# jthorborg/signalizer

Hardware: AMD Instinct MI355X
Metric: 32768-pt stereo STFT frames/sec (75% overlap); achieved HBM GB/s vs peak (higher is better)
Workload: dtype f32

## Files before the change

signalizer_amd/csrc/fft_scalar.hpp:

```cpp
#pragma once
#include "fft_common.hpp"

namespace sgz {

__device__ __forceinline__ v2 cmulScalar(v2 c, float2 w)
{
    const float t0 = c.x * w.x, t1 = c.x * w.y;
    return v2{__builtin_fmaf(-c.y, w.y, t0), __builtin_fmaf(c.y, w.x, t1)};
}
__device__ __forceinline__ float2 cmulScalar(float2 c, float2 w)
{
    const float t0 = c.x * w.x, t1 = c.x * w.y;
    return float2{__builtin_fmaf(-c.y, w.y, t0), __builtin_fmaf(c.y, w.x, t1)};
}
__device__ __forceinline__ float2 csqScalar(float2 w)
{
    const float d = w.x * w.x;
    return float2{__builtin_fmaf(-w.y, w.y, d), (w.x + w.x) * w.y};
}

template <int LR, int S, int BASE, int NREG>
__device__ __forceinline__ void ditStage(v2 (&c)[NREG])
{
    constexpr int n = 1 << LR, m = 1 << S, h = m / 2;
#pragma unroll
    for (int k0 = 0; k0 < n; k0 += m) {
#pragma unroll
        for (int j = 0; j < h; ++j) {
            const int ia = BASE + brev(k0 + j, LR), ib = BASE + brev(k0 + j + h, LR);
            const v2 a = c[ia], b = c[ib];
            const int tw = j * (32 / m);
            if (tw == 0) { c[ia] = a + b; c[ib] = a - b; }
            else if (tw == 8) { c[ia] = v2{a.x + b.y, a.y - b.x}; c[ib] = v2{a.x - b.y, a.y + b.x}; }
            else if (tw < 8) {
                const float cs = cos32(tw), sn = sin32(tw);
                const float pr = __builtin_fmaf(b.y, sn, __builtin_fmaf(b.x, cs, a.x));
                const float pi = __builtin_fmaf(b.x, -sn, __builtin_fmaf(b.y, cs, a.y));
                c[ia] = v2{pr, pi};
                c[ib] = v2{__builtin_fmaf(2.f, a.x, -pr), __builtin_fmaf(2.f, a.y, -pi)};
            } else {
                const float cs = cos32(tw - 8), sn = sin32(tw - 8);
                const float pr = __builtin_fmaf(b.x, -sn, __builtin_fmaf(b.y, cs, a.x));
                const float pi = __builtin_fmaf(b.y, -sn, __builtin_fmaf(b.x, -cs, a.y));
                c[ia] = v2{pr, pi};
                c[ib] = v2{__builtin_fmaf(2.f, a.x, -pr), __builtin_fmaf(2.f, a.y, -pi)};
            }
        }
    }
}

template <int LR, int BASE, int NREG, int FIRST = 1>
__device__ __forceinline__ void ditScalar(v2 (&c)[NREG])
{
    if constexpr (FIRST <= 1) ditStage<LR, 1, BASE>(c);
    if constexpr (FIRST <= 2 && LR >= 2) ditStage<LR, 2, BASE>(c);
    if constexpr (LR >= 3) ditStage<LR, 3, BASE>(c);
    if constexpr (LR >= 4) ditStage<LR, 4, BASE>(c);
    if constexpr (LR >= 5) ditStage<LR, 5, BASE>(c);
}

__device__ __forceinline__ void bflyPackedLow(v2 &a, v2 &b, v2 k)
{
    v2 t, p, q;
    asm("v_pk_fma_f32 %0, %1, %2, %3 op_sel_hi:[1,0,1]" : "=v"(t) : "v"(b), "s"(k), "v"(a));
    asm("v_pk_fma_f32 %0, %1, %2, %3 op_sel:[1,1,0] op_sel_hi:[0,1,1] neg_hi:[1,0,0]" : "=v"(p) : "v"(b), "s"(k), "v"(t));
    asm("v_pk_fma_f32 %0, %1, 2.0, %2 op_sel_hi:[1,0,1] neg_lo:[0,0,1] neg_hi:[0,0,1]" : "=v"(q) : "v"(a), "v"(p));
    a = p; b = q;
}
__device__ __forceinline__ void bflyPackedHigh(v2 &a, v2 &b, v2 k)
{
    v2 t, p, q;
    asm("v_pk_fma_f32 %0, %1, %2, %3 op_sel:[1,0,0] op_sel_hi:[0,0,1] neg_hi:[1,0,0]" : "=v"(t) : "v"(b), "s"(k), "v"(a));
    asm("v_pk_fma_f32 %0, %1, %2, %3 op_sel:[0,1,0] op_sel_hi:[1,1,1] neg_lo:[1,0,0] neg_hi:[1,0,0]" : "=v"(p) : "v"(b), "s"(k), "v"(t));
    asm("v_pk_fma_f32 %0, %1, 2.0, %2 op_sel_hi:[1,0,1] neg_lo:[0,0,1] neg_hi:[0,0,1]" : "=v"(q) : "v"(a), "v"(p));
    a = p; b = q;
}
__device__ __forceinline__ void bflyPackedRot(v2 &a, v2 &b)
{
    v2 p, q;
    asm("v_pk_add_f32 %0, %1, %2 op_sel:[0,1] op_sel_hi:[1,0] neg_hi:[0,1]" : "=v"(p) : "v"(a), "v"(b));
    asm("v_pk_add_f32 %0, %1, %2 op_sel:[0,1] op_sel_hi:[1,0] neg_lo:[0,1]" : "=v"(q) : "v"(a), "v"(b));
    a = p; b = q;
}

template <bool UNIT_A>
__device__ __forceinline__ void bflyPackedFusedTw(v2 &a, v2 &b, v2 ta, v2 tb)
{
    v2 u = a, t, p, q;
    if constexpr (!UNIT_A) {
        v2 m;
        asm("v_pk_mul_f32 %0, %1, %2 op_sel:[0,0] op_sel_hi:[1,0]" : "=v"(m) : "v"(a), "v"(ta));
        asm("v_pk_fma_f32 %0, %1, %2, %3 op_sel:[1,1,0] op_sel_hi:[0,1,1] neg_lo:[1,0,0]" : "=v"(u) : "v"(a), "v"(ta), "v"(m));
    }
    asm("v_pk_fma_f32 %0, %1, %2, %3 op_sel:[0,0,0] op_sel_hi:[1,0,1]" : "=v"(t) : "v"(b), "v"(tb), "v"(u));
    asm("v_pk_fma_f32 %0, %1, %2, %3 op_sel:[1,1,0] op_sel_hi:[0,1,1] neg_lo:[1,0,0]" : "=v"(p) : "v"(b), "v"(tb), "v"(t));
    asm("v_pk_fma_f32 %0, %1, 2.0, %2 op_sel_hi:[1,0,1] neg_lo:[0,0,1] neg_hi:[0,0,1]" : "=v"(q) : "v"(u), "v"(p));
    a = p; b = q;
}

template <int LR, int S, int BASE, int NREG>
__device__ __forceinline__ void ditStagePacked(v2 (&c)[NREG])
{
    constexpr int n = 1 << LR, m = 1 << S, h = m / 2;
#pragma unroll
    for (int k0 = 0; k0 < n; k0 += m) {
#pragma unroll
        for (int j = 0; j < h; ++j) {
            const int ia = BASE + brev(k0 + j, LR), ib = BASE + brev(k0 + j + h, LR);
            const int tw = j * (32 / m);
            if (tw == 0) { const v2 a = c[ia], b = c[ib]; c[ia] = a + b; c[ib] = a - b; }
            else if (tw == 8) bflyPackedRot(c[ia], c[ib]);
            else if (tw < 8) bflyPackedLow(c[ia], c[ib], v2{cos32(tw), sin32(tw)});
            else bflyPackedHigh(c[ia], c[ib], v2{cos32(tw - 8), sin32(tw - 8)});
        }
    }
}
template <int LR, int BASE, int NREG, int FIRST = 1>
__device__ __forceinline__ void ditPacked(v2 (&c)[NREG])
{
    if constexpr (FIRST <= 1) ditStagePacked<LR, 1, BASE>(c);
    if constexpr (FIRST <= 2 && LR >= 2) ditStagePacked<LR, 2, BASE>(c);
    if constexpr (LR >= 3) ditStagePacked<LR, 3, BASE>(c);
    if constexpr (LR >= 4) ditStagePacked<LR, 4, BASE>(c);
    if constexpr (LR >= 5) ditStagePacked<LR, 5, BASE>(c);
}

}
```

signalizer_amd/csrc/spectrum_real.hip:

```cpp
#include <algorithm>

#include "real_common.hpp"

#ifdef SGZ_DEBUG
#define RCLK(slot)                                                                                                     \
    do {                                                                                                               \
        if (prm.phaseClock && (tid & 63) == 0 && unit == long(prm.clkUnit)) prm.phaseClock[16 * (tid >> 6) + (slot)] = __builtin_readcyclecounter(); \
    } while (0)
#define RTRACE(which)                                                                                                  \
    do {                                                                                                               \
        if (prm.phaseClock && prm.clkUnit == 0xffffu && tid == 0) {                                                    \
            unsigned long long *t = prm.phaseClock + 256 + 4 * unit;                                                   \
            t[which] = __builtin_amdgcn_s_memrealtime();                                                               \
            if (which == 0) { t[2] = __builtin_amdgcn_s_getreg(4 | (31 << 11)); t[3] = __builtin_amdgcn_s_getreg(20 | (31 << 11)) | (static_cast<unsigned long long>(blockIdx.x) << 32); } \
        }                                                                                                              \
    } while (0)
#else
#define RCLK(slot) do { } while (0)
#define RTRACE(which) do { } while (0)
#endif

namespace sgz {

template <int R1, int LR1, int BASE, int Q = 0>
__device__ __forceinline__ void e1WriteRun(uint32_t wa, const v2 (&c)[32])
{
    if constexpr (Q < R1) { ldsWrite64<(Q & 15) * 512 * 8>(wa + uint32_t(Q >> 4) * 65536u, c[BASE + brev(Q, LR1)]); e1WriteRun<R1, LR1, BASE, Q + 1>(wa, c); }
}

template <int R1, int LR1, int Q = 0>
__device__ __forceinline__ void e1WritePairRun(uint32_t wa, const v2 (&c)[32])
{
    if constexpr (Q < R1) { ldsWrite128<(Q & 15) * 512 * 8>(wa + uint32_t(Q >> 4) * 65536u, c[brev(Q, LR1)], c[R1 + brev(Q, LR1)]); e1WritePairRun<R1, LR1, Q + 1>(wa, c); }
}

template <int R, int R1, int U, int LR1, int u = 0>
__device__ __forceinline__ void pass1Columns(v2 (&c)[R])
{
    if constexpr (u < U) {
        ditPacked<LR1, u * R1>(c);
        pass1Columns<R, R1, U, LR1, u + 1>(c);
    }
}

constexpr float kRotA1Cm1 = -0x1.3bd3ccp-24f, kRotA1Sin = 0x1.921fb4p-12f;
constexpr float kRotA4Cm1 = -0x1.3bd3c8p-20f, kRotA4Sin = 0x1.921faap-10f;
__device__ __forceinline__ float4 rotatePhaseForward(const float4 ph, const float cm1, const float sn)
{
    const v2 pc = v2{ph.x, ph.y}, ps = v2{ph.z, ph.w};
    const v2 kc = v2{cm1, cm1}, ks = v2{sn, sn};
    const v2 c2 = __builtin_elementwise_fma(pc, kc, __builtin_elementwise_fma(ps, -ks, pc));
    const v2 s2 = __builtin_elementwise_fma(ps, kc, __builtin_elementwise_fma(pc, ks, ps));
    return float4{c2.x, c2.y, s2.x, s2.y};
}
__device__ __forceinline__ float2 rotateTwiddle(const float2 w, const float cm1, const float sn)
{
    const v2 v = v2{w.x, w.y}, sw = v2{w.y, w.x};
    const v2 r = __builtin_elementwise_fma(v, v2{cm1, cm1}, __builtin_elementwise_fma(sw, v2{sn, -sn}, v));
    return float2{r.x, r.y};
}

__device__ __forceinline__ void windowPairCos(v2 &lo, v2 &hi, const int a32, const v2 pc, const v2 ps, const v2 p0)
{
    v2 t = pc;
    if (a32 != 0) {
        const v2 k = v2{cos32(a32), sin32(a32)};
        v2 m;
        asm("v_pk_mul_f32 %0, %1, %2 op_sel:[0,1] op_sel_hi:[1,1]" : "=v"(m) : "v"(ps), "s"(k));
        asm("v_pk_fma_f32 %0, %1, %2, %3 op_sel:[0,0,0] op_sel_hi:[1,0,1] neg_lo:[0,0,1] neg_hi:[0,0,1]" : "=v"(t) : "v"(pc), "s"(k), "v"(m));
    }
    v2 wa, wb;
    asm("v_pk_add_f32 %0, %1, %2" : "=v"(wa) : "v"(t), "s"(p0));
    asm("v_pk_add_f32 %0, %1, %2 neg_lo:[1,0] neg_hi:[1,0]" : "=v"(wb) : "v"(t), "s"(p0));
    lo = lo * wa;
    hi = hi * wb;
}

template <int LR1, int MIX, typename P>
__device__ __forceinline__ void realMapSettle(const P &prm, float *lds, const int tid, const int side, const long task, const long self,
                                              const ChunkTables &tb, ChunkMap<(1 << (LR1 + 5))> &mapper, float *re, float *ce, float *spec)
{
    constexpr int R = 32, R1 = 1 << LR1, T = R1 * R, M = R1 * R * R, N = 2 * M;
    constexpr bool MONO = MIX == 1 || MIX == 3;
    const ChannelIndex at{N, side ? M : 0};
    [[maybe_unused]] const long unit = MONO ? task : self;
    if (prm.binsOut) {
        float *dst = prm.binsOut + size_t(task) * (N + 1) + (side ? M : 0);
        for (int i = tid; i <= M; i += T)
            if (MONO || i != (side ? 0 : M)) dst[i] = lds[chunkPos(i)];
    }
    if (!MONO && (prm.lowCount[0] + prm.lowCount[1]) && tid < kLowBins) prm.low[size_t(self) * kLowBins + tid] = lds[at(side ? N - tid : tid)];
    RCLK(8);
    mapper.run(tb, at, lds, re, ce, prm.invSize, tid);
    RCLK(9);
    RTRACE(1);
    if (MONO) {
        if (prm.mapped && prm.lowCount[0]) {
            float *out = prm.mapped + size_t(task) * prm.P;
            for (uint32_t i = tid; i < prm.lowCount[0]; i += T) {
                const uint32_t x = prm.lowPixels[i];
                out[x] = complexDcPixel(prm.recsFull[x], prm.weights, prm.invSize, N, prm.mode,
                                        [&](int k) { return k >= N ? 0.f : lds[chunkPos(k)]; },
                                        [&](int sl) { return make_float2(spec[2 * sl], spec[2 * sl + 1]); });
            }
        }
        return;
    }
}

[[maybe_unused]] __device__ __forceinline__ void setWavePriority(const uint32_t p)
{
    if (p != 0u) { if (p == 1u) __builtin_amdgcn_s_setprio(1); else if (p == 2u) __builtin_amdgcn_s_setprio(2); else __builtin_amdgcn_s_setprio(3); }
}

constexpr uint32_t kNyHopRows = 4;
template <int LR1, bool PRIO, bool SHARE>
__device__ __forceinline__ void nyquistUnit(const RealParams &prm, float *lds, const uint32_t light, const int tid)
{
    constexpr int LR = 5, R = 32, R1 = 1 << LR1, RR = R * R;
    static_assert(LR1 == 4, "the Nyquist workgroups mirror the two-columns-per-thread form (N = 32768)");
    [[maybe_unused]] const long unit = 2 * long(light) + 1;
    RTRACE(0);
#ifdef SGZ_IMAGE_PRIO
    if constexpr (PRIO) setWavePriority(prm.prioNy);
#endif
#ifdef SGZ_SCHED_SWEEP
    for (uint32_t k = 0; k < prm.nyDelay; ++k) __builtin_amdgcn_s_sleep(16);
#endif
    const uint32_t F = prm.nyFrames, perPair = uint32_t(prm.frames) / F + (uint32_t(prm.frames) % F != 0u);
    const uint32_t pair = light / perPair, f0 = (light - pair * perPair) * F;
    const uint32_t f1 = f0 + F < uint32_t(prm.frames) ? f0 + F : uint32_t(prm.frames);
    const float *X0 = prm.planar + size_t(2 * pair + 1) * prm.chStride;
    const uint32_t lane16 = uint32_t(tid) * 16u;
    const float4 ph[2] = {ldg(prm.winPhase, lane16 * 2u), ldg(prm.winPhase + 1, lane16 * 2u)};
    const v2 p0 = v2{prm.winP0, prm.winP0};
    v2 *lds2 = reinterpret_cast<v2 *>(lds);
    auto columnSum = [&](v2 (&c)[R1], const int u) {
        const v2 pc = v2{ph[u].x, ph[u].y}, ps = v2{ph[u].z, ph[u].w};
#pragma unroll
        for (int j = 0; j < R1 / 2; ++j) windowPairCos(c[j], c[j + R1 / 2], j * (32 / R1), pc, ps, p0);
        ditPacked<LR1, 0>(c);
        lds2[2 * tid + u] = c[0];
    };
    auto tree2 = [&]() {
        if (tid < R) {
            v2 s[R];
#pragma unroll
            for (int h = 0; h < R; ++h) s[h] = lds2[tid + R * h];
            ditPacked<LR, 0>(s);
            lds2[RR + tid] = s[0];
        }
    };
    auto tree3 = [&](const uint32_t f) {
        if (tid == 0) {
            v2 s[R];
#pragma unroll
            for (int r = 0; r < R; ++r) s[r] = lds2[RR + r];
            const float4 *tab = prm.tw2Full;
#pragma unroll
            for (int i = 0; i < R / 4; ++i) {
                const float4 wa = tab[i], wb = tab[i + R / 4];
                if (i == 0) bflyPackedFusedTw<true>(s[0], s[R / 2], v2{1.f, 0.f}, v2{wb.x, wb.y});
                else bflyPackedFusedTw<false>(s[2 * i], s[2 * i + R / 2], v2{wa.x, wa.y}, v2{wb.x, wb.y});
                bflyPackedFusedTw<false>(s[2 * i + 1], s[2 * i + 1 + R / 2], v2{wa.z, wa.w}, v2{wb.z, wb.w});
            }
            ditPacked<LR, 0, R, 2>(s);
            prm.ny[((size_t(f) * prm.C + pair) << 1) | 1u] = 2.f * (s[0].x - s[0].y);
        }
    };
    constexpr uint32_t HOPROWS = kNyHopRows;
    if (SHARE && f1 - f0 > 1u && prm.hop == HOPROWS * 2u * uint32_t(RR)) {
        typedef float v4 __attribute__((ext_vector_type(4)));
        v4 raw[R1];
        {
            const float *X = X0 + size_t(f0) * prm.hop;
#pragma unroll
            for (int j = 0; j < R1; ++j) raw[j] = ldgPinned<v4>(X, uint32_t(RR * j) * 8u, lane16);
        }
        for (uint32_t f = f0; f < f1; ++f) {
#pragma unroll
            for (int u = 0; u < 2; ++u) {
                v2 c[R1];
#pragma unroll
                for (int j = 0; j < R1; ++j) c[j] = u ? v2{raw[j].z, raw[j].w} : v2{raw[j].x, raw[j].y};
                columnSum(c, u);
            }
            if (f + 1u < f1) {
                const float *X = X0 + size_t(f + 1u) * prm.hop;
#pragma unroll
                for (int j = 0; j < R1 - int(HOPROWS); ++j) raw[j] = raw[j + int(HOPROWS)];
#pragma unroll
                for (int j = R1 - int(HOPROWS); j < R1; ++j) raw[j] = ldgPinned<v4>(X, uint32_t(RR * j) * 8u, lane16);
            }
            constexpr int PARK = R1 - int(HOPROWS);
            v4 *park = reinterpret_cast<v4 *>(lds + 4 * RR) + (tid & 63);
            if (__builtin_amdgcn_readfirstlane(tid) < 64) {
                __syncthreads();
#pragma unroll
                for (int j = 0; j < PARK; ++j) park[64 * j] = raw[j];
                tree2();
                __syncthreads();
                tree3(f);
#pragma unroll
                for (int j = 0; j < PARK; ++j) raw[j] = park[64 * j];
            } else {
                __syncthreads();
                __syncthreads();
            }
        }
        RTRACE(1);
        return;
    }
    for (uint32_t f = f0; f < f1; ++f) {
        const float *X = X0 + size_t(f) * prm.hop;
#pragma unroll
        for (int u = 0; u < 2; ++u) {
            v2 c[R1];
#pragma unroll
            for (int j = 0; j < R1; ++j) c[j] = ldgPinned<v2>(X, uint32_t(RR * j) * 8u + 8u * u, lane16);
            columnSum(c, u);
        }
        __syncthreads();
        tree2();
        __syncthreads();
        tree3(f);
    }
    RTRACE(1);
}

template <int LR1, bool WCOS, int MIX = 0, bool PRIO = false>
__global__ void __launch_bounds__(1 << (LR1 + 5), 4) stftRealKernel(const RealParams launchPrm)
{
    constexpr int LR = 5, R = 32, R1 = 1 << LR1, T = R1 * R, RR = R * R, M = R1 * RR, N = 2 * M, U = R / R1;
    constexpr bool MONO = MIX == 1 || MIX == 3;
    constexpr bool SIDE0 = MIX == 4;
    constexpr bool mixed = MIX == 2 || MIX == 3;
    constexpr int PADSTRIDE = chunkPos(T);
    constexpr int ROW = R + 2, TILE = R * ROW;
    constexpr int XFLOATS = realXFloats(M);
    static_assert((T / R) * TILE <= XFLOATS, "the exchange-2 tiles end below the twiddle table");
    constexpr int TAB = (XFLOATS + 3) & ~3;
    extern __shared__ __attribute__((aligned(16))) float lds[];
    const int tid0 = threadIdx.x;

    constexpr bool WALK = LR1 == 5 && MIX == 0 && WCOS;
    const uint32_t heavyUnits = SIDE0 ? uint32_t(launchPrm.frames) * launchPrm.C : gridDim.x;
    if constexpr (SIDE0) {
        if (blockIdx.x >= heavyUnits) { nyquistUnit<LR1, PRIO, PRIO>(launchPrm, lds, blockIdx.x - heavyUnits, opaque(tid0)); return; }
    }
    const uint32_t totalUnits = WALK ? uint32_t(launchPrm.frames) * launchPrm.C * 2u : heavyUnits;
    uint32_t walkIndex = blockIdx.x;
    UnitId uid = unitOfIndex<MONO || SIDE0>(launchPrm, walkIndex, totalUnits, SIDE0 && launchPrm.mateAdjacent != 0u);
    [[maybe_unused]] bool firstUnit = true;
    [[maybe_unused]] uint32_t prioEarly = 0u, prioLate = 0u, prioEnds = 0u;
    if constexpr (LR1 == 4) {
        const uint32_t cus = launchPrm.roundSize >> 1;
#ifndef SGZ_STAGGER
#define SGZ_STAGGER 5
#endif
        if (cus && !launchPrm.pipelined && gridDim.x >= 2u * cus && blockIdx.x >= cus && blockIdx.x < 2u * cus) {
#pragma unroll
            for (int k = 0; k < SGZ_STAGGER; ++k) __builtin_amdgcn_s_sleep(32);
        }
#ifdef SGZ_SCHED_SWEEP
        else if (SIDE0 && blockIdx.x >= cus) {
            for (uint32_t k = 0; k < launchPrm.mateDelay; ++k) __builtin_amdgcn_s_sleep(16);
        }
#endif
#ifndef SGZ_NO_PRIO
        if (cus && !launchPrm.pipelined && gridDim.x > 2u * cus && gridDim.x <= 3u * cus) {
#else
        if (false) {
#endif
            const uint32_t generation = blockIdx.x / cus;
            if (generation == 0u) __builtin_amdgcn_s_setprio(2); else if (generation == 1u) __builtin_amdgcn_s_setprio(1); else __builtin_amdgcn_s_setprio(3);
        }
#ifdef SGZ_IMAGE_PRIO
        if constexpr (PRIO) {
#ifdef SGZ_SCHED_SWEEP
            const uint32_t rolePrio = blockIdx.x >= cus ? launchPrm.prioMate : blockIdx.x + cus < heavyUnits ? launchPrm.prioFirst : 0u;
            const uint32_t scope = launchPrm.prioScope;
#else
            const uint32_t rolePrio = blockIdx.x >= cus ? (launchPrm.prioMate ? uint32_t(SGZ_PRIO_MATE) : 0u)
                                                        : blockIdx.x + cus < heavyUnits ? (launchPrm.prioFirst ? uint32_t(SGZ_PRIO_FIRST) : 0u) : 0u;
            constexpr uint32_t scope = SGZ_PRIO_SCOPE;
#endif
            prioEarly = (scope == 0u || scope == 3u) ? rolePrio : 0u;
            prioLate = (scope == 1u || scope == 2u) ? rolePrio : 0u;
            prioEnds = (scope & 1u) ? rolePrio : 0u;
            prioEarly = __builtin_amdgcn_readfirstlane(prioEarly); prioLate = __builtin_amdgcn_readfirstlane(prioLate); prioEnds = __builtin_amdgcn_readfirstlane(prioEnds);
        }
#endif
    }
    constexpr bool PAIRED = U == 2;
    constexpr int COLSTEP = PAIRED ? 1 : T, COLLANE = PAIRED ? 2 : 1;
    constexpr bool FRONT = LR1 >= 4 && !mixed && WCOS;
#ifdef SGZ_DIET
    constexpr bool DIET = PAIRED && FRONT && LR1 == 4;
#else
    constexpr bool DIET = false;
#endif
    [[maybe_unused]] float4 phase[U];
    [[maybe_unused]] float2 twA[U], twB[U];
    [[maybe_unused]] float4 tw2piece, tw2tail;
    v2 c[R];
    for (;;) {
    typename ParamsOf<WALK>::T &prm = *ParamsOf<WALK>::get(launchPrm);
    auto samplesOf = [&](const UnitId &u) {
        const int firstCh = MONO ? (prm.mode == SGZ_CH_RIGHT ? 1 : 0) : (mixed ? 0 : u.side);
        return prm.planar + size_t(2 * u.pair + firstCh) * prm.chStride + size_t(u.frame) * prm.hop;
    };
    auto elemOf = [&](int e) { const int u = e / R1, j = e % R1; return (PAIRED ? u : T * u) + RR * j; };
    auto requestSamples = [&](const float *X, const int tid, auto partTag) {
        constexpr int part = decltype(partTag)::value;
        const uint32_t lane8 = uint32_t(tid) * (PAIRED ? 16u : 8u);
        if constexpr (PAIRED) {
            typedef float v4 __attribute__((ext_vector_type(4)));
#pragma unroll
            for (int j = 0; j < R1; ++j) { const v4 xv = ldgPinned<v4>(X, uint32_t(RR * j) * 8u, lane8); c[j] = v2{xv.x, xv.y}; c[R1 + j] = v2{xv.z, xv.w}; }
        } else {
#pragma unroll
            for (int i = 0; i < R; ++i)
                if (part == 0 || ((i >> 3) & 1) == part - 1) c[i] = ldgPinned<v2>(X, uint32_t(elemOf(i)) * 8u, lane8);
        }
    };
    auto requestTables = [&](const int tid) {
        if constexpr (FRONT) {
            if constexpr (WALK) tw2piece = prm.tw2Full[tid < kTw2Floats / 4 ? tid : 0];
#pragma unroll
            for (int u = 0; u < (DIET ? 1 : U); ++u) {
                if (WCOS) phase[u] = ldg(prm.winPhase + COLSTEP * u, uint32_t(tid) * 16u * COLLANE);
                twA[u] = ldg(prm.tw1 + (COLSTEP * u), uint32_t(tid) * 8u * COLLANE);
                twB[u] = ldg(prm.tw1 + (COLSTEP * u + 3 * RR), uint32_t(tid) * 8u * COLLANE);
            }
            if constexpr (!WALK) { if (tid < kTw2Floats / 4) tw2piece = prm.tw2Full[tid]; }
            if (T < kTw2Floats / 4 && tid < kTw2Floats / 4 - T) tw2tail = prm.tw2Full[T + tid];
        }
    };
    if constexpr (WALK) {
        if (firstUnit) requestSamples(samplesOf(uid), tid0, std::integral_constant<int, 1>{});
        firstUnit = false;
    }
    const int tid = WALK ? opaque(tid0) : tid0;
    const int slot = tid >> 6, half = (tid >> 5) & 1, l = tid & 31, group = tid >> 5;
    const int q1 = half ? (slot == 0 ? R1 / 2 : R1 - slot) : slot;
    const int ix = half ? R - 1 - l : l;
    const uint32_t lane8 = uint32_t(tid) * (PAIRED ? 16u : 8u);
    [[maybe_unused]] const long unit = MONO ? long(uid.task) : long(uid.self);
    const int side = SIDE0 ? 0 : uid.side, pair = uid.pair;
    const long task = uid.task, frame = uid.frame, self = uid.self;

    const uint32_t maxSlots = prm.chunkSlots[0] > prm.chunkSlots[1] ? prm.chunkSlots[0] : prm.chunkSlots[1];
    const ChunkTables tb{prm.chunkEnds + side * T, prm.chunkReBase + side * T,
                         reinterpret_cast<const uint2 *>(prm.chunkRec) + size_t(side) * prm.P, prm.recs + size_t(side) * prm.P, prm.weights12,
                         prm.mapped ? prm.mapped + (size_t(task) * (MONO ? 1 : 2) + side) * prm.P : nullptr,
                         MONO ? nullptr : prm.nyBest + size_t(self) * 64, int(prm.fixFrom[side]), int(prm.P), side != 0,
#ifdef SGZ_DEBUG
                         (prm.phaseClock && unit == long(prm.clkUnit)) ? prm.phaseClock : nullptr};
#else
                         nullptr};
#endif
    const ChannelIndex at{N, side ? M : 0};
    float *re = lds + XFLOATS, *ce = re + maxSlots + 1;
    const int SCRATCH = XFLOATS + int(realExtraFloats(maxSlots, T, LR1 >= 4));
    float *spec = lds + SCRATCH + 2 * R;
    ChunkMap<T> mapper;

    RCLK(0);
    RTRACE(0);
    if constexpr (LR1 >= 4 && !FRONT) {
        for (int i = tid; i < kTw2Floats / 4; i += T) reinterpret_cast<float4 *>(lds + TAB)[i] = prm.tw2Full[i];
    }
    {
        const float *X = samplesOf(uid);
        if constexpr (WALK) {
            requestTables(tid);
            __builtin_amdgcn_sched_barrier(0);
            requestSamples(X, tid, std::integral_constant<int, 2>{});
            __builtin_amdgcn_sched_barrier(0);
            if (tid < kTw2Floats / 4) reinterpret_cast<float4 *>(lds + TAB)[tid] = tw2piece;
        } else {
            requestSamples(X, tid, std::integral_constant<int, 0>{});
            requestTables(tid);
        }
        if constexpr (FRONT) __builtin_amdgcn_sched_barrier(0);
#ifdef SGZ_IMAGE_PRIO
        if constexpr (PRIO) setWavePriority(prioEarly);
#endif
        if (mixed) {
            const float *Y = X + prm.chStride;
            const float sgn = (MONO ? prm.mode == SGZ_CH_SIDE : side == 1) ? -1.f : 1.f;
            constexpr int YB = (LR1 == 5 || (PAIRED && !WCOS)) ? 4 : 8;
#pragma unroll
            for (int b0 = 0; b0 < R; b0 += YB) {
                float2 y[YB];
#pragma unroll
                for (int i = 0; i < YB; ++i) y[i] = ldg(reinterpret_cast<const float2 *>(Y) + elemOf(b0 + i), lane8);
#pragma unroll
                for (int i = 0; i < YB; ++i) c[b0 + i] = v2{c[b0 + i].x + sgn * y[i].x, c[b0 + i].y + sgn * y[i].y};
                __builtin_amdgcn_sched_barrier(0);
            }
        }
        if (WCOS) {
            const v2 p0 = v2{prm.winP0, prm.winP0};
#pragma unroll
            for (int u = 0; u < U; ++u) {
                const float4 ph = (DIET && u == 1) ? rotatePhaseForward(phase[0], kRotA1Cm1, kRotA1Sin)
                                  : FRONT ? phase[u] : ldg(prm.winPhase + COLSTEP * u, uint32_t(tid) * 16u * COLLANE);
                const v2 pc = v2{ph.x, ph.y}, ps = v2{ph.z, ph.w};
#pragma unroll
                for (int j = 0; j < R1 / 2; ++j) {
                    constexpr int S32 = 32 / R1;
                    const int a32 = j * S32;
                    const int i = u * R1 + j, i2 = i + R1 / 2;
                    if constexpr (LR1 == 3) {
                        const float cj = cos32(a32), sj = sin32(a32);
                        const float te = a32 == 0 ? ph.x : ph.x * cj - ph.z * sj, to = a32 == 0 ? ph.y : ph.y * cj - ph.w * sj;
                        c[i] = v2{c[i].x * (prm.winP0 + te), c[i].y * (prm.winP0 + to)};
                        c[i2] = v2{c[i2].x * (prm.winP0 - te), c[i2].y * (prm.winP0 - to)};
                        continue;
                    }
                    windowPairCos(c[i], c[i2], a32, pc, ps, p0);
                }
            }
        } else {
            constexpr int B = LR1 >= 4 ? 4 : 8;
            float2 wa[B], wb[B];
#pragma unroll
            for (int i = 0; i < B; ++i) wa[i] = ldg(reinterpret_cast<const float2 *>(prm.window) + elemOf(i), lane8);
#pragma unroll
            for (int b0 = 0; b0 < R; b0 += 2 * B) {
#pragma unroll
                for (int i = 0; i < B; ++i) wb[i] = ldg(reinterpret_cast<const float2 *>(prm.window) + elemOf(b0 + B + i), lane8);
                __builtin_amdgcn_sched_barrier(0);
#pragma unroll
                for (int i = 0; i < B; ++i) { c[b0 + i] = v2{c[b0 + i].x * wa[i].x, c[b0 + i].y * wa[i].y}; asm volatile("" : "+v"(c[b0 + i])); }
                if (b0 + 2 * B < R) {
#pragma unroll
                    for (int i = 0; i < B; ++i) wa[i] = ldg(reinterpret_cast<const float2 *>(prm.window) + elemOf(b0 + 2 * B + i), lane8);
                }
                __builtin_amdgcn_sched_barrier(0);
#pragma unroll
                for (int i = 0; i < B; ++i) { c[b0 + B + i] = v2{c[b0 + B + i].x * wb[i].x, c[b0 + B + i].y * wb[i].y}; asm volatile("" : "+v"(c[b0 + B + i])); }
            }
        }
    }
    if (mixed) {
#pragma unroll
        for (int i = 0; i < R; ++i) c[i] = v2{c[i].x * 0.5f, c[i].y * 0.5f};
    }
    __builtin_amdgcn_sched_barrier(0);
    RCLK(13);
    pass1Columns<R, R1, U, LR1>(c);
#ifdef SGZ_IMAGE_PRIO
    if constexpr (PRIO) setWavePriority(prioLate);
#endif
#pragma unroll
    for (int u = 0; u < U; ++u) {
        constexpr int NB = R1 / 4 - 1;
        float2 a[3], b[NB];
        auto sq = [](float2 w) { return float2{w.x * w.x - w.y * w.y, 2.f * w.x * w.y}; };
        auto mul = [](float2 p, float2 q) { return float2{p.x * q.x - p.y * q.y, p.x * q.y + p.y * q.x}; };
        if (DIET && u == 1) {
            a[0] = rotateTwiddle(twA[0], kRotA1Cm1, kRotA1Sin);
            if (NB > 0) b[0] = rotateTwiddle(twB[0], kRotA4Cm1, kRotA4Sin);
        } else {
            a[0] = FRONT ? twA[u] : ldg(prm.tw1 + (COLSTEP * u), uint32_t(tid) * 8u * COLLANE);
            if (NB > 0) b[0] = FRONT ? twB[u] : ldg(prm.tw1 + (COLSTEP * u + 3 * RR), uint32_t(tid) * 8u * COLLANE);
        }
        a[1] = sq(a[0]); a[2] = mul(a[1], a[0]);
#pragma unroll
        for (int i = 1; i < NB; ++i) b[i] = (i & 1) ? sq(b[i / 2]) : mul(b[i - 1], b[0]);
#pragma unroll
        for (int q = 1; q < R1; ++q) {
            const int qa = q >> 2, qb = q & 3;
            v2 w;
            if (qa == 0) w = v2{a[qb - 1].x, a[qb - 1].y};
            else if (qb == 0) w = v2{b[qa - 1].x, b[qa - 1].y};
            else w = cmul(v2{b[qa - 1].x, b[qa - 1].y}, v2{a[qb - 1].x, a[qb - 1].y});
            const int i = u * R1 + brev(q, LR1);
            c[i] = cmul(c[i], w);
        }
    }
    RCLK(1);
    {
        v2 *lds2 = reinterpret_cast<v2 *>(lds);
        auto writeRound = [&](int r) {
            if constexpr (PAIRED) {
                if ((tid >> 8) == r) e1WritePairRun<R1, LR1>(ldsAddress(lds2 + ((2 * tid) & 511)), c);
                return;
            }
#pragma unroll
            for (int u = 0; u < U; ++u) {
                const int col = COLLANE * tid + COLSTEP * u;
                if ((col >> 9) == r) {
#ifndef SGZ_E1_PAIRED_WRITES
                    const uint32_t wa = ldsAddress(lds2 + (col & 511));
                    if (u == 0) e1WriteRun<R1, LR1, 0>(wa, c);
                    else if (u == 1) e1WriteRun<R1, LR1, (U > 1 ? R1 : 0)>(wa, c);
                    else if (u == 2) e1WriteRun<R1, LR1, (U > 2 ? 2 * R1 : 0)>(wa, c);
                    else e1WriteRun<R1, LR1, (U > 3 ? 3 * R1 : 0)>(wa, c);
#else
#pragma unroll
                    for (int q = 0; q < R1; ++q) lds2[q * 512 + (col & 511)] = c[u * R1 + brev(q, LR1)];
#endif
                }
            }
        };
        const int rd = q1 * 512 + ix;
        v2 lo[R / 2];
        if constexpr (FRONT && !WALK) {
            if (tid < kTw2Floats / 4) reinterpret_cast<float4 *>(lds + TAB)[tid] = tw2piece;
            if (T < kTw2Floats / 4 && tid < kTw2Floats / 4 - T) reinterpret_cast<float4 *>(lds + TAB)[T + tid] = tw2tail;
        }
        writeRound(0);
        ldsBarrier();
        const uint32_t rdAddr = ldsAddress(lds2 + rd);
        ldsReadRun64<16, R * 8>(lo, rdAddr);
        ldsReadsDone(lo);
        ldsBarrier();
        writeRound(1);
        ldsBarrier();
        {
            v2 hi[16];
            ldsReadRun64<16, R * 8>(hi, rdAddr);
            ldsReadsDone(hi);
#pragma unroll
            for (int h = 0; h < R / 2; ++h) { c[h + R / 2] = hi[h]; c[h] = lo[h]; }
        }
    }
    ldsBarrier();
    RCLK(2);
    constexpr bool EARLYTAB = WALK || (LR1 == 4 && FRONT);
    [[maybe_unused]] float2 wkEarly;
    if constexpr (EARLYTAB) {
        wkEarly = ldg(prm.twPost, uint32_t(q1 + R1 * ix) * 8u);
        mapper.prefetch(tb, tid);
    }
    ditPacked<LR, 0>(c);
#ifndef SGZ_NO_TW_FUSE
    constexpr bool TWFUSE = LR1 >= 4;
#else
    constexpr bool TWFUSE = false;
#endif
#ifndef SGZ_LATE_DEAD_BARRIER
    constexpr bool EARLYDEAD = TWFUSE && LR1 == 5;
#else
    constexpr bool EARLYDEAD = false;
#endif
    if constexpr (LR1 >= 4 && !TWFUSE) {
        const float4 *tab = reinterpret_cast<const float4 *>(lds + TAB + ix * kTw2Row);
#pragma unroll
        for (int i = 0; i < R / 2; ++i) {
            const float4 w = tab[i];
            if (i > 0) c[brev(2 * i, LR)] = cmul(c[brev(2 * i, LR)], v2{w.x, w.y});
            c[brev(2 * i + 1, LR)] = cmul(c[brev(2 * i + 1, LR)], v2{w.z, w.w});
        }
    } else if constexpr (!TWFUSE) {
        TwFactors<LR> tw;
        tw.load(prm.tw2, ix, R);
        tw.apply(c);
    }
    RCLK(3);
    {
        const int tile = group * TILE;
        const uint32_t rowAddr = ldsAddress(lds + tile + ix * ROW);
#pragma unroll
        for (int q2 = 0; q2 < R; ++q2) lds[tile + q2 * ROW + ix] = c[brev(q2, LR)].x;
        __builtin_amdgcn_fence(__ATOMIC_RELEASE, "workgroup");
        __builtin_amdgcn_wave_barrier();
        __builtin_amdgcn_fence(__ATOMIC_ACQUIRE, "workgroup");
        { v2 t[16]; ldsReadRun64<16, 8>(t, rowAddr); ldsReadsDone(t);
#pragma unroll
          for (int j = 0; j < R / 2; ++j) { c[2 * j].x = t[j].x; c[2 * j + 1].x = t[j].y; } }
        __builtin_amdgcn_fence(__ATOMIC_RELEASE, "workgroup");
        __builtin_amdgcn_wave_barrier();
#pragma unroll
        for (int q2 = 0; q2 < R; ++q2) lds[tile + q2 * ROW + ix] = c[brev(q2, LR)].y;
        __builtin_amdgcn_fence(__ATOMIC_RELEASE, "workgroup");
        __builtin_amdgcn_wave_barrier();
        __builtin_amdgcn_fence(__ATOMIC_ACQUIRE, "workgroup");
        { v2 t[16]; ldsReadRun64<16, 8>(t, rowAddr); ldsReadsDone(t);
#pragma unroll
          for (int j = 0; j < R / 2; ++j) { c[2 * j].y = t[j].x; c[2 * j + 1].y = t[j].y; } }
    }
    RCLK(4);
    float2 wk;
    if constexpr (EARLYTAB) wk = wkEarly; else wk = ldg(prm.twPost, uint32_t(q1 + R1 * ix) * 8u);
    if constexpr (TWFUSE) {
        const float4 *tab = reinterpret_cast<const float4 *>(lds + TAB + ix * kTw2Row);
#pragma unroll
        for (int i = 0; i < R / 4; ++i) {
            const float4 wa = tab[i], wb = tab[i + R / 4];
            if (i == 0) bflyPackedFusedTw<true>(c[0], c[R / 2], v2{1.f, 0.f}, v2{wb.x, wb.y});
            else bflyPackedFusedTw<false>(c[2 * i], c[2 * i + R / 2], v2{wa.x, wa.y}, v2{wb.x, wb.y});
            bflyPackedFusedTw<false>(c[2 * i + 1], c[2 * i + 1 + R / 2], v2{wa.z, wa.w}, v2{wb.z, wb.w});
        }
        if constexpr (EARLYDEAD) ldsBarrier();
        ditPacked<LR, 0, R, 2>(c);
    } else {
        ditPacked<LR, 0>(c);
    }
    RCLK(5);
    const int kc = q1 + R1 * ix;
    if (tid == 0) {
#pragma unroll
        for (int m3 = 0; m3 < R; ++m3) {
            lds[SCRATCH + 2 * m3] = c[brev(m3, LR)].x;
            lds[SCRATCH + 2 * m3 + 1] = c[brev(m3, LR)].y;
        }
        if (!MONO) prm.ny[self] = 2.f * (c[0].x - c[0].y);
    }
    float fixA = 0.f, fixB = 0.f;
    if (tid <= R / 2) {
        __builtin_amdgcn_fence(__ATOMIC_RELEASE, "workgroup");
        __builtin_amdgcn_wave_barrier();
        __builtin_amdgcn_fence(__ATOMIC_ACQUIRE, "workgroup");
        if (tid >= 1) {
            const int m3 = tid;
            const v2 a = v2{lds[SCRATCH + 2 * m3], lds[SCRATCH + 2 * m3 + 1]};
            const v2 b = v2{lds[SCRATCH + 2 * (R - m3)], lds[SCRATCH + 2 * (R - m3) + 1]};
            const float cs = cospif(float(m3) * (1.0f / 32.0f)), sn = sinpif(float(m3) * (1.0f / 32.0f));
            fixA = realBinMag(a, b, v2{cs, -sn});
            fixB = realBinMag(b, a, v2{-cs, -sn});
        } else {
            fixA = lds[SCRATCH] + lds[SCRATCH + 1];
            if (MONO) { fixA = __builtin_fabsf(fixA); fixB = lds[SCRATCH] - lds[SCRATCH + 1]; }
        }
    }
    float magA[R / 2], magB[R / 2];
    [[maybe_unused]] UnitId nextUid = uid;
    [[maybe_unused]] bool more = false;
    [[maybe_unused]] const float *nextX = nullptr;
    [[maybe_unused]] v2 nextRows[R / 2];
    if constexpr (WALK) {
        const uint32_t nextIndex = walkIndex + gridDim.x;
        more = nextIndex < totalUnits;
        if (more) { nextUid = unitOfIndex<MONO>(prm, nextIndex, totalUnits); walkIndex = nextIndex; }
        nextX = samplesOf(nextUid);
    }
    {
        const int lane = int(__builtin_amdgcn_mbcnt_hi(~0u, __builtin_amdgcn_mbcnt_lo(~0u, 0u)));
        int plane = lane ^ R;
        if (slot == 0) plane = (lane & ~(R - 1)) | (half ? R - 1 - l : ((R - l) & (R - 1)));
        plane <<= 2;
        auto partnerOf = [&](float v) {
            return __builtin_bit_cast(float, __builtin_amdgcn_ds_bpermute(plane, __builtin_bit_cast(int, v)));
        };
#ifdef SGZ_MIRROR_BPERMUTE
        if (true) {
#else
        if (slot == 0) {
#endif
#pragma unroll
            for (int m3 = 0; m3 < R / 2; ++m3) { const int ip = brev(R - 1 - m3, LR); c[ip] = v2{partnerOf(c[ip].x), partnerOf(c[ip].y)}; }
        } else {
#pragma unroll
            for (int m3 = 0; m3 < R / 2; m3 += 4)
                halfWaveExchange4(c[brev(R - 1 - m3, LR)], c[brev(R - 2 - m3, LR)], c[brev(R - 3 - m3, LR)], c[brev(R - 4 - m3, LR)]);
        }
#pragma unroll
        for (int m3 = 0; m3 < R / 2; ++m3) {
            const int i = brev(m3, LR), ip = brev(R - 1 - m3, LR);
            const v2 a = c[i];
            const v2 b = c[ip];
            const v2 w = m3 == 0 ? v2{wk.x, wk.y} : cmulConjK(v2{wk.x, wk.y}, v2{cos64(m3), sin64(m3)});
            v2 E, D, t, O, re2, im2, sq;
            asm("v_pk_add_f32 %0, %1, %2 neg_hi:[0,1]" : "=v"(E) : "v"(a), "v"(b));
            asm("v_pk_add_f32 %0, %1, %2 neg_lo:[0,1]" : "=v"(D) : "v"(a), "v"(b));
            asm("v_pk_mul_f32 %0, %1, %2 op_sel:[0,1] op_sel_hi:[1,1]" : "=v"(t) : "v"(w), "v"(D));
            asm("v_pk_fma_f32 %0, %1, %2, %3 op_sel:[1,0,0] op_sel_hi:[0,0,1] neg_hi:[1,0,0]" : "=v"(O) : "v"(w), "v"(D), "v"(t));
            asm("v_pk_add_f32 %0, %1, %2 op_sel:[0,0] op_sel_hi:[0,0] neg_hi:[0,1]" : "=v"(re2) : "v"(E), "v"(O));
            asm("v_pk_add_f32 %0, %1, %2 op_sel:[1,1] op_sel_hi:[1,1] neg_hi:[0,1]" : "=v"(im2) : "v"(E), "v"(O));
            sq = re2 * re2;
            asm("v_pk_fma_f32 %0, %1, %1, %2" : "=v"(sq) : "v"(im2), "v"(sq));
            const float pr = re2.x, mr = re2.y, pi = im2.x, mi = im2.y;
            magA[m3] = __builtin_amdgcn_sqrtf(sq.x);
            magB[m3] = __builtin_amdgcn_sqrtf(sq.y);
            if constexpr (WALK) {
                const int row = m3 < 8 ? m3 : m3 + 8;
                nextRows[m3] = ldgPinned<v2>(nextX, uint32_t(elemOf(row)) * 8u, lane8);
            }
            if (MONO && m3 == 0 && prm.lowCount[0] && kc >= 1 && kc <= 8) {
                spec[2 * (8 - kc)] = pr; spec[2 * (8 - kc) + 1] = -pi;
                if (kc < 8) { spec[2 * (8 + kc)] = mr; spec[2 * (8 + kc) + 1] = mi; }
            }
        }
    }
    if constexpr (WALK) {
#pragma unroll
        for (int m3 = 0; m3 < R / 2; ++m3) c[m3 < 8 ? m3 : m3 + 8] = nextRows[m3];
    }
    RCLK(6);
#ifdef SGZ_IMAGE_PRIO
    if constexpr (PRIO) { if (prioEnds != 0u) __builtin_amdgcn_s_setprio(0); }
#endif
    if (!MONO && side == 0 && q1 == 1 && ix == 0) magB[0] *= 0.5f;
    if constexpr (WALK) mapper.arrived(); else if constexpr (!EARLYTAB) mapper.prefetch(tb, tid);
    if constexpr (!EARLYDEAD) ldsBarrier();
    {
        const int up = chunkPos(kc), down = chunkPos(M - kc);
        int lowest = down - (R / 2 - 1) * PADSTRIDE;
        asm volatile("" : "+v"(lowest));
        float *pu = lds + up, *pd = lds + lowest;
        if (side == 0) {
#pragma unroll
            for (int m3 = 0; m3 < R / 2; ++m3) { pu[m3 * PADSTRIDE] = magA[m3]; pd[(R / 2 - 1 - m3) * PADSTRIDE] = magB[m3]; }
        } else {
#pragma unroll
            for (int m3 = 0; m3 < R / 2; ++m3) { pd[(R / 2 - 1 - m3) * PADSTRIDE] = magA[m3]; pu[m3 * PADSTRIDE] = magB[m3]; }
        }
    }
    if (tid <= R / 2) {
        auto put = [&](int k, float v) { const int i = side ? M - k : k; lds[chunkPos(i)] = v; };
        if (tid >= 1) {
            put(T * tid, fixA);
            if (tid != R / 2) put(T * (R - tid), fixB);
        } else {
            put(0, fixA);
            if (MONO) { spec[16] = fixB; spec[17] = 0.f; }
            put(M, MONO ? fixB : 0.f);
        }
    }
    *reinterpret_cast<float2 *>(lds + chunkPos(32 * tid) + 32) = float2{0.f, 0.f};
    if (tid < 16) lds[chunkPos(M) + 1 + tid] = 0.f;
    ldsBarrier();
    RCLK(7);
    realMapSettle<LR1, MIX>(prm, lds, tid, side, task, self, tb, mapper, re, ce, spec);
    if constexpr (!WALK) break;
    else {
        if (!more) break;
        uid = nextUid;
        ldsBarrier();
    }
    }
}

template <int LR1>
__global__ void __launch_bounds__(1 << (LR1 + 5)) realMapFromBinsKernel(const RealParams prm)
{
    constexpr int R = 32, R1 = 1 << LR1, T = R1 * R, M = R1 * R * R, N = 2 * M;
    constexpr int XFLOATS = realXFloats(M);
    extern __shared__ __attribute__((aligned(16))) float lds[];
    const int tid = threadIdx.x;
    const long unit = blockIdx.x;
    const int side = int(unit & 1);
    const long task = unit >> 1;
    const long self = (task << 1) | side;
    const uint32_t maxSlots = prm.chunkSlots[0] > prm.chunkSlots[1] ? prm.chunkSlots[0] : prm.chunkSlots[1];
    const ChunkTables tb{prm.chunkEnds + side * T, prm.chunkReBase + side * T,
                         reinterpret_cast<const uint2 *>(prm.chunkRec) + size_t(side) * prm.P, prm.recs + size_t(side) * prm.P, prm.weights12,
                         prm.mapped ? prm.mapped + (size_t(task) * 2 + side) * prm.P : nullptr, prm.nyBest + size_t(self) * 64, int(prm.fixFrom[side]), int(prm.P), side != 0, nullptr};
    float *re = lds + XFLOATS, *ce = re + maxSlots + 1;
    ChunkMap<T> mapper;
    mapper.prefetch(tb, tid);
    const float *src = prm.binsIn + size_t(task) * (N + 1) + (side ? M : 0);
    for (int i = tid; i <= M; i += T) lds[chunkPos(i)] = (i == (side ? 0 : M)) ? 0.f : src[i];
    *reinterpret_cast<float2 *>(lds + chunkPos(32 * tid) + 32) = float2{0.f, 0.f};
    if (tid < 16) lds[chunkPos(M) + 1 + tid] = 0.f;
    if (tid == 0) prm.ny[self] = src[side ? 0 : M];
    __syncthreads();
    realMapSettle<LR1, 0>(prm, lds, tid, side, task, self, tb, mapper, re, ce, lds);
}

__host__ __device__ LateFix lateFixOf(const RealParams &prm)
{
    return LateFix{prm.ny, prm.nyBest, prm.fixFrom[0], prm.fixFrom[1], prm.P, prm.invSize, prm.binsIn ? 1u : 0u};
}
__global__ void __launch_bounds__(256) realLateKernel(const RealParams prm, const int N, const uint32_t nTop)
{
#pragma clang fp contract(off)
    const long tasks = prm.frames * long(prm.C);
    const long item = long(blockIdx.x) * 256 + threadIdx.x;
    const long tops = tasks * 2 * nTop;
    const uint32_t nLow = prm.lowCount[0] + prm.lowCount[1];
    if (item < tops) {
        const long task = item / (2 * nTop);
        const int s = int((item / nTop) & 1);
        const uint32_t j = uint32_t(item % nTop);
        const LateFix lf = lateFixOf(prm);
        const uint32_t x = lf.fixFrom(s) + j;
        const bool top = x < prm.P && prm.mapped;
        float *px = prm.mapped + size_t(2 * task + s) * prm.P + (top ? x : 0u);
        const float own = top ? *px : 0.f;
        const float best = top ? lateBestSquare(lf, task, s, x) : 0.f;
        const float vM = lateNyquistBin(lf, task);
        if (s == 0 && j == 0 && prm.binsOut) prm.binsOut[size_t(task) * (N + 1) + N / 2] = vM;
        if (top) {
            const float v = lateNyquistPixel(lf, vM, best, own);
            if (v != own || !(own == own)) *px = v;
        }
    } else if (item < tops + tasks * nLow && prm.mapped) {
        const long task = (item - tops) / nLow;
        const uint32_t n = uint32_t((item - tops) % nLow);
        const int s = n < prm.lowCount[0] ? 0 : 1;
        const uint32_t x = prm.lowPixels[n];
        const PixelRec rec = prm.recsFull[size_t(s) * prm.P + x];
        const float *lowL = prm.low + size_t(2 * task) * kLowBins, *lowR = lowL + kLowBins;
        float acc = 0.f;
        int k = rec.a;
        for (int i = 0; i < rec.b; ++i) {
            const float v = k < kLowBins ? lowL[k] : lowR[N - k];
            acc = acc + v * prm.weights[rec.c + i];
            k = (k == N) ? 0 : k + 1;
        }
        prm.mapped[(size_t(2 * task + s)) * prm.P + x] = finishPixel<5>(prm.invSize * acc);
    }
}
hipError_t launchRealLate(const RealParams &prm, uint32_t N, hipStream_t stream)
{
    const long tasks = prm.frames * long(prm.C);
    if (tasks <= 0) return hipSuccess;
    uint32_t nTop = 1;
    for (int s = 0; s < 2; ++s) nTop = std::max(nTop, std::min(64u, prm.P - std::min(prm.P, prm.fixFrom[s])));
    const long items = tasks * 2 * nTop + tasks * long(prm.lowCount[0] + prm.lowCount[1]);
    hipLaunchKernelGGL(realLateKernel, dim3(unsigned((items + 255) / 256)), dim3(256), 0, stream, prm, int(N), nTop);
    return hipGetLastError();
}

__global__ void __launch_bounds__(256) finishPixelKernel(const float *x, float *y, size_t n)
{
    const size_t i = size_t(blockIdx.x) * blockDim.x + threadIdx.x;
    if (i < n) y[i] = finishPixel<5>(x[i]);
}
hipError_t launchFinishPixel(const float *x, float *y, size_t n, hipStream_t stream)
{
    if (n == 0) return hipSuccess;
    hipLaunchKernelGGL(finishPixelKernel, dim3(unsigned((n + 255) / 256)), dim3(256), 0, stream, x, y, n);
    return hipGetLastError();
}

hipError_t launchStftReal(const RealParams &prm, uint32_t N, hipStream_t stream)
{
    const bool mono = prm.mode != SGZ_CH_SEPARATE && prm.mode != SGZ_CH_MIDSIDE;
    const bool side0 = prm.nyFrames && N == 32768 && prm.mode == SGZ_CH_SEPARATE && prm.winPhase && prm.lateInNext && prm.mapped && !prm.binsOut &&
                       !prm.binsIn && prm.lowCount[0] + prm.lowCount[1] == 0;
    const long tasks = prm.frames * long(prm.C);
    const long units = side0 ? tasks + long(prm.C) * ((prm.frames + prm.nyFrames - 1) / prm.nyFrames) : tasks * (mono ? 1 : 2);
    if (units <= 0) return hipSuccess;
    const uint32_t M = N / 2, T = M / 32;
    const uint32_t maxSlots = std::max(prm.chunkSlots[0], prm.chunkSlots[1]);
    const size_t ldsBytes = (size_t(realXFloats(int(M))) + realExtraFloats(maxSlots, T, N >= 32768) + 64 + (mono ? 2 * kSpecBins : 0)) * 4;
    static size_t granted[29][64] = {};
    const bool wcos = prm.winPhase != nullptr;
    if (prm.binsIn) {
        if (mono) return hipErrorNotSupported;
        auto inject = [&](auto kern, int slot, unsigned threads) -> hipError_t {
            if (hipError_t e = grantLds(reinterpret_cast<const void *>(kern), ldsBytes, granted[slot]); e != hipSuccess) return e;
            hipLaunchKernelGGL(kern, dim3(unsigned(units)), dim3(threads), ldsBytes, stream, prm);
            return launchRealLate(prm, N, stream);
        };
        if (N == 32768) return inject(&realMapFromBinsKernel<4>, 24, 512);
        if (N == 16384) return inject(&realMapFromBinsKernel<3>, 25, 256);
        if (N == 65536) return inject(&realMapFromBinsKernel<5>, 26, 1024);
        return hipErrorNotSupported;
    }
    auto go = [&](auto kern, int slot, unsigned threads, size_t limit) -> hipError_t {
        if (ldsBytes > limit) return hipErrorInvalidValue;
        if (hipError_t e = grantLds(reinterpret_cast<const void *>(kern), ldsBytes, granted[slot]); e != hipSuccess) return e;
        const bool walk = N == 65536 && !mono && prm.mode == SGZ_CH_SEPARATE && wcos && prm.roundSize;
        hipLaunchKernelGGL(kern, dim3(unsigned(walk ? std::min<long>(units, long(prm.roundSize)) : units)), dim3(threads), ldsBytes, stream, prm);
        if (!mono && !prm.lateInNext) return launchRealLate(prm, N, stream);
        return hipSuccess;
    };
    hipError_t e;
    if (mono && (prm.mode == SGZ_CH_MERGE || prm.mode == SGZ_CH_SIDE)) {
        if (N == 32768) e = wcos ? go(&stftRealKernel<4, true, 3>, 18, 512, 80 * 1024) : go(&stftRealKernel<4, false, 3>, 19, 512, 80 * 1024);
        else if (N == 16384) e = wcos ? go(&stftRealKernel<3, true, 3>, 20, 256, 40 * 1024) : go(&stftRealKernel<3, false, 3>, 21, 256, 40 * 1024);
        else if (N == 65536) e = wcos ? go(&stftRealKernel<5, true, 3>, 22, 1024, 160 * 1024) : go(&stftRealKernel<5, false, 3>, 23, 1024, 160 * 1024);
        else return hipErrorNotSupported;
        if (e != hipSuccess) return e;
        return hipGetLastError();
    }
    if (mono) {
        if (N == 32768) e = wcos ? go(&stftRealKernel<4, true, 1>, 6, 512, 80 * 1024) : go(&stftRealKernel<4, false, 1>, 7, 512, 80 * 1024);
        else if (N == 16384) e = wcos ? go(&stftRealKernel<3, true, 1>, 8, 256, 40 * 1024) : go(&stftRealKernel<3, false, 1>, 9, 256, 40 * 1024);
        else if (N == 65536) e = wcos ? go(&stftRealKernel<5, true, 1>, 10, 1024, 160 * 1024) : go(&stftRealKernel<5, false, 1>, 11, 1024, 160 * 1024);
        else return hipErrorNotSupported;
        if (e != hipSuccess) return e;
        return hipGetLastError();
    }
    if (prm.mode == SGZ_CH_MIDSIDE) {
        if (N == 32768) e = wcos ? go(&stftRealKernel<4, true, 2>, 12, 512, 80 * 1024) : go(&stftRealKernel<4, false, 2>, 13, 512, 80 * 1024);
        else if (N == 16384) e = wcos ? go(&stftRealKernel<3, true, 2>, 14, 256, 40 * 1024) : go(&stftRealKernel<3, false, 2>, 15, 256, 40 * 1024);
        else if (N == 65536) e = wcos ? go(&stftRealKernel<5, true, 2>, 16, 1024, 160 * 1024) : go(&stftRealKernel<5, false, 2>, 17, 1024, 160 * 1024);
        else return hipErrorNotSupported;
        if (e != hipSuccess) return e;
        return hipGetLastError();
    }
#ifdef SGZ_IMAGE_PRIO
    if (side0 && ((prm.prioFirst | prm.prioMate | prm.prioNy) || (prm.nyFrames > 1u && prm.frames > 1 && prm.hop == kNyHopRows * 2048u)))
        e = go(&stftRealKernel<4, true, 4, true>, 28, 512, 80 * 1024);
    else
#endif
    if (side0) e = go(&stftRealKernel<4, true, 4>, 27, 512, 80 * 1024);
    else if (N == 32768) e = wcos ? go(&stftRealKernel<4, true>, 0, 512, 80 * 1024) : go(&stftRealKernel<4, false>, 1, 512, 80 * 1024);
    else if (N == 16384) e = wcos ? go(&stftRealKernel<3, true>, 4, 256, 40 * 1024) : go(&stftRealKernel<3, false>, 5, 256, 40 * 1024);
    else if (N == 65536) e = wcos ? go(&stftRealKernel<5, true>, 2, 1024, 160 * 1024) : go(&stftRealKernel<5, false>, 3, 1024, 160 * 1024);
    else return hipErrorNotSupported;
    if (e != hipSuccess) return e;
    return hipGetLastError();
}

}
```

Baseline: 14.97 million.

## Stream pass-1 DIT butterflies as bit-reversed sample loads arrive

For the LR1==4 paired front-loaded path, samples are requested in bit-reversed order and the radix-16 column FFT runs block by block as each pair of inputs arrives, with windowing applied per arrival. The window-phase loads are issued before the samples so they are ready early. The aim is to overlap global-load latency with butterfly arithmetic instead of waiting for all loads before pass 1. In exchange, the instruction schedule depends on the compiler honouring waitcnt granularity, and register pressure may rise.

New measurement: 15.14 million (median of 6 runs). 1.01x the previous value.

```diff
diff --git a/signalizer_amd/csrc/fft_scalar.hpp b/signalizer_amd/csrc/fft_scalar.hpp
--- a/signalizer_amd/csrc/fft_scalar.hpp
+++ b/signalizer_amd/csrc/fft_scalar.hpp
@@ -98,22 +98,26 @@
     a = p; b = q;
 }
 
+template <int LR, int S, int NREG>
+__device__ __forceinline__ void ditBlockPacked(v2 (&c)[NREG], const int base, const int k0)
+{
+    constexpr int m = 1 << S, h = m / 2;
+#pragma unroll
+    for (int j = 0; j < h; ++j) {
+        const int ia = base + brev(k0 + j, LR), ib = base + brev(k0 + j + h, LR);
+        const int tw = j * (32 / m);
+        if (tw == 0) { const v2 a = c[ia], b = c[ib]; c[ia] = a + b; c[ib] = a - b; }
+        else if (tw == 8) bflyPackedRot(c[ia], c[ib]);
+        else if (tw < 8) bflyPackedLow(c[ia], c[ib], v2{cos32(tw), sin32(tw)});
+        else bflyPackedHigh(c[ia], c[ib], v2{cos32(tw - 8), sin32(tw - 8)});
+    }
+}
 template <int LR, int S, int BASE, int NREG>
 __device__ __forceinline__ void ditStagePacked(v2 (&c)[NREG])
 {
-    constexpr int n = 1 << LR, m = 1 << S, h = m / 2;
+    constexpr int n = 1 << LR, m = 1 << S;
 #pragma unroll
-    for (int k0 = 0; k0 < n; k0 += m) {
-#pragma unroll
-        for (int j = 0; j < h; ++j) {
-            const int ia = BASE + brev(k0 + j, LR), ib = BASE + brev(k0 + j + h, LR);
-            const int tw = j * (32 / m);
-            if (tw == 0) { const v2 a = c[ia], b = c[ib]; c[ia] = a + b; c[ib] = a - b; }
-            else if (tw == 8) bflyPackedRot(c[ia], c[ib]);
-            else if (tw < 8) bflyPackedLow(c[ia], c[ib], v2{cos32(tw), sin32(tw)});
-            else bflyPackedHigh(c[ia], c[ib], v2{cos32(tw - 8), sin32(tw - 8)});
-        }
-    }
+    for (int k0 = 0; k0 < n; k0 += m) ditBlockPacked<LR, S>(c, BASE, k0);
 }
 template <int LR, int BASE, int NREG, int FIRST = 1>
 __device__ __forceinline__ void ditPacked(v2 (&c)[NREG])
@@ -125,4 +129,25 @@
     if constexpr (LR >= 5) ditStagePacked<LR, 5, BASE>(c);
 }
 
+template <int LR, int S, int NREG>
+__device__ __forceinline__ void ditBlocksEndingAt(v2 (&c)[NREG], const int base, const int end)
+{
+    if constexpr (S <= LR) {
+        constexpr int m = 1 << S;
+        if (end % m == 0) { ditBlockPacked<LR, S>(c, base, end - m); ditBlocksEndingAt<LR, S + 1>(c, base, end); }
+    }
 }
+template <int LR, int COLS, int STRIDE, int NREG, typename F>
+__device__ __forceinline__ void ditPackedByArrival(v2 (&c)[NREG], F &&arrived)
+{
+#pragma unroll
+    for (int i = 0; i < (1 << LR); i += 2) {
+#pragma unroll
+        for (int u = 0; u < COLS; ++u) {
+            arrived(u, brev(i, LR));
+            ditBlocksEndingAt<LR, 1>(c, u * STRIDE, i + 2);
+        }
+    }
+}
+
+}
diff --git a/signalizer_amd/csrc/spectrum_real.hip b/signalizer_amd/csrc/spectrum_real.hip
--- a/signalizer_amd/csrc/spectrum_real.hip
+++ b/signalizer_amd/csrc/spectrum_real.hip
@@ -300,6 +300,7 @@
 #else
     constexpr bool DIET = false;
 #endif
+    constexpr bool STREAM = LR1 == 4 && PAIRED && FRONT && !DIET;
     [[maybe_unused]] float4 phase[U];
     [[maybe_unused]] float2 twA[U], twB[U];
     [[maybe_unused]] float4 tw2piece, tw2tail;
@@ -317,19 +318,26 @@
         if constexpr (PAIRED) {
             typedef float v4 __attribute__((ext_vector_type(4)));
 #pragma unroll
-            for (int j = 0; j < R1; ++j) { const v4 xv = ldgPinned<v4>(X, uint32_t(RR * j) * 8u, lane8); c[j] = v2{xv.x, xv.y}; c[R1 + j] = v2{xv.z, xv.w}; }
+            for (int i = 0; i < R1; ++i) {
+                const int j = STREAM ? brev(i, LR1) : i;
+                const v4 xv = ldgPinned<v4>(X, uint32_t(RR * j) * 8u, lane8); c[j] = v2{xv.x, xv.y}; c[R1 + j] = v2{xv.z, xv.w};
+            }
         } else {
 #pragma unroll
             for (int i = 0; i < R; ++i)
                 if (part == 0 || ((i >> 3) & 1) == part - 1) c[i] = ldgPinned<v2>(X, uint32_t(elemOf(i)) * 8u, lane8);
         }
+    };
+    auto requestPhases = [&](const int tid) {
+#pragma unroll
+        for (int u = 0; u < (DIET ? 1 : U); ++u) phase[u] = ldg(prm.winPhase + COLSTEP * u, uint32_t(tid) * 16u * COLLANE);
     };
     auto requestTables = [&](const int tid) {
         if constexpr (FRONT) {
             if constexpr (WALK) tw2piece = prm.tw2Full[tid < kTw2Floats / 4 ? tid : 0];
+            if constexpr (WCOS && !STREAM) requestPhases(tid);
 #pragma unroll
             for (int u = 0; u < (DIET ? 1 : U); ++u) {
-                if (WCOS) phase[u] = ldg(prm.winPhase + COLSTEP * u, uint32_t(tid) * 16u * COLLANE);
                 twA[u] = ldg(prm.tw1 + (COLSTEP * u), uint32_t(tid) * 8u * COLLANE);
                 twB[u] = ldg(prm.tw1 + (COLSTEP * u + 3 * RR), uint32_t(tid) * 8u * COLLANE);
             }
@@ -380,6 +388,7 @@
             __builtin_amdgcn_sched_barrier(0);
             if (tid < kTw2Floats / 4) reinterpret_cast<float4 *>(lds + TAB)[tid] = tw2piece;
         } else {
+            if constexpr (STREAM) { requestPhases(tid); __builtin_amdgcn_sched_barrier(0); }
             requestSamples(X, tid, std::integral_constant<int, 0>{});
             requestTables(tid);
         }
@@ -403,8 +412,17 @@
         }
         if (WCOS) {
             const v2 p0 = v2{prm.winP0, prm.winP0};
-#pragma unroll
-            for (int u = 0; u < U; ++u) {
+            if constexpr (STREAM) {
+                ditPackedByArrival<LR1, U, R1>(c, [&](const int u, const int j) __attribute__((always_inline)) {
+#ifdef SGZ_DEBUG
+                    if (u == 0 && j == 0) { asm volatile("" : "+v"(c[0]), "+v"(c[R1 / 2])); RCLK(14); }
+                    if (u == 0 && j == R1 / 2 - 1) { asm volatile("" : "+v"(c[R1 / 2 - 1]), "+v"(c[R1 - 1])); RCLK(15); }
+#endif
+                    windowPairCos(c[u * R1 + j], c[u * R1 + j + R1 / 2], j * (32 / R1), v2{phase[u].x, phase[u].y}, v2{phase[u].z, phase[u].w}, p0);
+                });
+            }
+#pragma unroll
+            for (int u = 0; u < (STREAM ? 0 : U); ++u) {
                 const float4 ph = (DIET && u == 1) ? rotatePhaseForward(phase[0], kRotA1Cm1, kRotA1Sin)
                                   : FRONT ? phase[u] : ldg(prm.winPhase + COLSTEP * u, uint32_t(tid) * 16u * COLLANE);
                 const v2 pc = v2{ph.x, ph.y}, ps = v2{ph.z, ph.w};
@@ -451,7 +469,7 @@
     }
     __builtin_amdgcn_sched_barrier(0);
     RCLK(13);
-    pass1Columns<R, R1, U, LR1>(c);
+    if constexpr (!STREAM) pass1Columns<R, R1, U, LR1>(c);
 #ifdef SGZ_IMAGE_PRIO
     if constexpr (PRIO) setWavePriority(prioLate);
 #endif
```
